# hinike/cairo

Measured on AMD Instinct MI355X. Metric: encoded Mpixels/s (p-frame, q=16) at 1/2/4/8 MI355X; bit-exact vs ref, higher is better.
Workload: dtype int16

## Files before the change

### cairo_amd/__init__.py

```python
from __future__ import annotations

import ctypes
import os
from dataclasses import dataclass

import numpy as np

_HERE = os.path.dirname(os.path.abspath(__file__))
LIB_PATH = os.path.join(_HERE, "_lib", "libcairo_amd.so")

BLOCK_DESC = np.dtype(
    [
        ("block_type", "<u4"),
        ("prediction_target", "u1"),
        ("pad", "u1"),
        ("motion_x", "<i2"),
        ("motion_y", "<i2"),
        ("sp_pred", "u1"),
        ("sp_amount", "u1"),
        ("sp_index", "u1"),
        ("q_index", "u1"),
        ("variance", "<i2"),
    ]
)
# ... 373 lines not shown
    def __del__(self):
        try:
            self.close()
        except Exception:
            pass

    @property
    def stages(self) -> int:
        return int(self.L.cairo_ctx_stages(self.h))

    def submit(self, rgb, index: int, inter: bool, quality: int, on_device: bool = False,
               fmt: int = FMT_RGB24, pitch: int = 0, src_size=None, crop=None) -> int:
        t = ctypes.c_int()
        if src_size is not None or crop is not None:
            if src_size is None:
                raise ValueError("crop needs src_size")
            s = _source(src_size, crop)
            ptr = _scaled_source_ptr(rgb, on_device, fmt, src_size, pitch)
            _ck(self.L.cairo_ctx_submit_scaled(self.h, ptr, fmt, pitch, ctypes.byref(s), index, int(inter), quality,
                                               ctypes.byref(t)), "cairo_ctx_submit_scaled")
            return t.value
        ptr = rgb if on_device else _host_frame_fmt(rgb, fmt, self.width, self.height, pitch)
        if fmt == FMT_RGB24 and not pitch:
            _ck(
                self.L.cairo_ctx_submit(self.h, ptr, int(on_device), index, int(inter), quality, ctypes.byref(t)),
                "cairo_ctx_submit",
            )
        else:
            _ck(self.L.cairo_ctx_submit_fmt(self.h, ptr, int(on_device), fmt, pitch, index, int(inter), quality,
                                            ctypes.byref(t)), "cairo_ctx_submit_fmt")
        if not on_device:
            self._keep[t.value] = rgb
        return t.value

    def wait(self, ticket: int, copy: bool = True) -> FrameOutputs:
        r = _FrameResult()
        st = self.L.cairo_ctx_wait(self.h, ticket, ctypes.byref(r))
        if st != EVX_SUCCESS:
            raise CairoError("cairo_ctx_wait", st, self.timeout_info() if st == EVX_ERROR_HARDWAREFAIL else None)
        self._keep.pop(ticket, None)
        return self._outputs(r, copy)

    ACCT_FIELDS = ("coder_tasks", "coder_total", "coder_group_wait", "coder_window", "coder_search", "coder_inter",
                   "coder_dequeue", "coder_mbs", "helper_tasks", "helper_total", "helper_wait", "helper_deblock",
                   "helper_search", "helper_catchup", "helper_dequeue", "helper_chunks",
                   "win_bytes", "win_spec_unused_bytes", "zero_mv_bytes", "gran_poll_bytes", "rec_poll_bytes",
                   "win_stages", "searched_tasks", "inter_tasks", "coder_xform", "coder_publish", "coder_drain",
                   "coder_vm0", "coder_records", "coder_prebarrier", "coder_store_tail",
                   "search_eval", "search_barrier", "search_select", "subpel_eval", "subpel_barrier",
                   "subpel_select", "db_inputs", "db_filter", "db_write",
                   "search_passes", "search_mbs_2pass", "search_mbs_3pass", "search_mbs_4pass",
                   "coder_xform_copy", "coder_copy_mbs", "coder_xform_coded", "coder_coded_mbs",
                   "helper_carry", "carry_bytes",
                   "coder_prologue_fresh", "coder_prologue_records", "helper_group_start")

    def read_acct(self, reset: bool = False) -> dict:
        w = np.zeros(len(self.ACCT_FIELDS), np.uint64)
        _ck(self.L.cairo_ctx_read_acct(self.h, _ptr(w), len(w), int(reset)), "cairo_ctx_read_acct")
        return {k: int(w[i]) for i, k in enumerate(self.ACCT_FIELDS)}

    def timeout_info(self) -> dict | None:
        w = np.zeros(16, np.int32)
        _ck(self.L.cairo_ctx_timeout_info(self.h, _ptr(w), 16), "cairo_ctx_timeout_info")
        if not w[0]:
            return None
        d = {k: int(w[i]) for i, k in enumerate(TIMEOUT_FIELDS)}
        d["kind"] = WAIT_KINDS.get(d["kind"], str(d["kind"]))
        d["seen"] = (d.pop("seen_hi") & 0xFFFFFFFF) << 32 | (d.pop("seen_lo") & 0xFFFFFFFF)
        return d

    def _outputs(self, r, copy: bool) -> FrameOutputs:
        ny, nc = r.wa * r.ha, (r.wa // 2) * (r.ha // 2)
        mbs = r.wmb * r.hmb
        has_coef = bool(r.coef_y)
        feed = _view(r.feed, np.uint32, (r.feed_bits + 31) // 32) if r.feed_status == FEED_VALID else None
        out = FrameOutputs(
            _view(r.block_table, BLOCK_DESC, mbs),
            _view(r.coef_y, np.int16, ny).reshape(r.ha, r.wa) if has_coef else None,
            _view(r.coef_u, np.int16, nc).reshape(r.ha // 2, r.wa // 2) if has_coef else None,
            _view(r.coef_v, np.int16, nc).reshape(r.ha // 2, r.wa // 2) if has_coef else None,
            feed, int(r.feed_bits), int(r.feed_status),
        )
        if copy:
            cp = lambda a: None if a is None else a.copy()
            out = FrameOutputs(cp(out.table), cp(out.coef_y), cp(out.coef_u), cp(out.coef_v), cp(out.feed),
                               out.feed_bits, out.feed_status)
        return out

    def set_outputs(self, outputs: int) -> None:
        _ck(self.L.cairo_ctx_set_outputs(self.h, outputs), "cairo_ctx_set_outputs")

    def fetch_coef(self, ticket: int):
        r = _FrameResult()
        _ck(self.L.cairo_ctx_fetch_coef(self.h, ticket, ctypes.byref(r)), "cairo_ctx_fetch_coef")
        ny, nc = self.wa * self.ha, (self.wa // 2) * (self.ha // 2)
        return (_view(r.coef_y, np.int16, ny).reshape(self.ha, self.wa).copy(),
                _view(r.coef_u, np.int16, nc).reshape(self.ha // 2, self.wa // 2).copy(),
                _view(r.coef_v, np.int16, nc).reshape(self.ha // 2, self.wa // 2).copy())

    def set_metrics(self, sse: bool = True, ssim: bool = True, keep_recon: bool = False, flags: int | None = None) -> None:
        if flags is None:
            flags = (METRIC_SSE if sse else 0) | (METRIC_SSIM if ssim else 0) | (KEEP_RECON if keep_recon else 0)
        _ck(self.L.cairo_ctx_set_metrics(self.h, flags), "cairo_ctx_set_metrics")

    def frame_metrics(self, ticket: int) -> dict:
        m = _FrameMetrics()
        _ck(self.L.cairo_ctx_frame_metrics(self.h, ticket, ctypes.byref(m)), "cairo_ctx_frame_metrics")
# ... 531 lines not shown
```

### cairo_amd/csrc/kernels.h

```cpp
#pragma once

#include <hip/hip_runtime.h>
#include <stddef.h>
#include <stdint.h>

#include "evx_defs.h"

namespace cairo {

struct PlaneSet {
  int16_t* y;
  int16_t* u;
  int16_t* v;
};

__host__ __device__ inline PlaneSet ring_slot(int16_t* base, size_t slot_elems, int wa, int ha,
                                              int k) {
  PlaneSet p;
  p.y = base + (size_t)k * slot_elems;
  p.u = p.y + (size_t)wa * ha;
  p.v = p.u + (size_t)(wa / 2) * (ha / 2);
  return p;
}

// ... 3 lines not shown
__host__ __device__ inline uint32_t pack_inter_desc(const BlockDesc& d) {
  return (d.block_type & 7u) | ((uint32_t)(d.prediction_target & 3) << 3) | ((uint32_t)(d.sp_pred & 1) << 5) |
         ((uint32_t)(d.sp_amount & 1) << 6) | ((uint32_t)(d.sp_index & 15) << 7) |
         (((uint32_t)d.motion_x & 0x7Fu) << 11) | (((uint32_t)d.motion_y & 0x7Fu) << 18);
}
__host__ __device__ inline BlockDesc unpack_inter_desc(uint32_t w) {
  BlockDesc d;
  d.block_type = w & 7u;
  d.prediction_target = (uint8_t)((w >> 3) & 3);
  d.pad = 0;
  d.sp_pred = (uint8_t)((w >> 5) & 1);
  d.sp_amount = (uint8_t)((w >> 6) & 1);
  d.sp_index = (uint8_t)((w >> 7) & 15);
  d.motion_x = (int16_t)((int32_t)(w << 14) >> 25);
  d.motion_y = (int16_t)((int32_t)(w << 7) >> 25);
  d.q_index = 0;
  d.variance = 0;
  return d;
}

constexpr int kStampPhases = 12;
constexpr int kDbStamps = 256;
constexpr int kIStamps = 12;
__host__ __device__ inline size_t stamp_frame_words(int wmb, int hmb) {
  return (size_t)wmb * hmb * kStampPhases + (size_t)hmb * kDbStamps;
}

struct TimeoutInfo {
  static constexpr int kKind = 0;
  static constexpr int kEpoch = 1;
  static constexpr int kIndex = 2;
  static constexpr int kRow = 3;
  static constexpr int kMember = 4;
  static constexpr int kNeed = 5;
  static constexpr int kOn = 6;
  static constexpr int kSeenLo = 7;
  static constexpr int kSeenHi = 8;
  static constexpr int kClaim = 9;
  static constexpr int kWords = 16;
};
enum TimeoutKind : int32_t {
  kWaitRecords = 1,
  kWaitGranule = 2,
  kWaitPrevProgress = 3,
  kWaitRowAbove = 4,
  kWaitBatch = 5,
  kWaitInjected = 6,
  kWaitHostMark = 9,
};

#ifndef CAIRO_ACCT
#define CAIRO_ACCT 0
#endif
constexpr int kAcctShards = 64, kAcctWords = 53;
struct Acct {
  static constexpr int kCoderTasks = 0, kCoderTotal = 1, kCoderGroupWait = 2, kCoderWindow = 3, kCoderSearch = 4,
                       kCoderInter = 5, kCoderDequeue = 6, kCoderMBs = 7;
  static constexpr int kHelperTasks = 8, kHelperTotal = 9, kHelperWait = 10, kHelperDeblock = 11, kHelperSearch = 12,
                       kHelperCatchup = 13, kHelperDequeue = 14, kHelperChunks = 15;
  static constexpr int kWinBytes = 16, kWinSpecUnused = 17, kZeroMvBytes = 18, kGranPollBytes = 19,
                       kRecPollBytes = 20, kWinStages = 21, kSearchedTasks = 22, kInterTasks = 23;
  static constexpr int kCoderXform = 24, kCoderPublish = 25, kCoderDrain = 26;
  static constexpr int kCoderVm0 = 27, kCoderRecords = 28, kCoderPreBarrier = 29;
  static constexpr int kCoderStoreTail = 30;
  static constexpr int kSrchEval = 31, kSrchBarrier = 32, kSrchSelect = 33, kSubEval = 34, kSubBarrier = 35,
                       kSubSelect = 36;
  static constexpr int kDbInputs = 37, kDbFilter = 38, kDbWrite = 39;
  static constexpr int kSrchPasses = 40, kSrchPasses2 = 41, kSrchPasses3 = 42, kSrchPasses4 = 43;
  static constexpr int kCoderXformCopy = 44, kCoderCopyMBs = 45, kCoderXformCoded = 46, kCoderCodedMBs = 47;
  static constexpr int kHelperCarry = 48, kCarryBytes = 49;
  static constexpr int kCoderProFresh = 50, kCoderProRecords = 51, kHelperGroupStart = 52;
};

#ifndef CAIRO_MAX_BATCH
#define CAIRO_MAX_BATCH 48
#endif
constexpr int kMaxBatch = CAIRO_MAX_BATCH;
constexpr int kMaxGroup = 16;
constexpr int kMaxPush = kMaxRing;

struct FrameDesc {
  const uint8_t* rgb;
  const uint8_t* host_rgb;
  int index;
  int inter;
  int quality;
  uint32_t epoch;
  int slot;
  int decode;
  PlaneSet recon[kMaxRing];
  PlaneSet stale;
  PlaneSet coef;
  PlaneSet push[kMaxPush];
  int npush;
  PlaneSet coef_prev;
  uint64_t* progress;
  const uint64_t* prev_progress;
  const uint64_t* prev2_progress;
  int sys;
  int member;
  const BlockDesc* host_table;
  const int16_t* host_coef;
};

struct alignas(64) FrameArgs {
  int wa, ha;
  int wmb, hmb;
  uint32_t epoch;
  int nrec;
  BlockDesc* inter_desc;
  PlaneSet in;
  uint64_t* granules;
  PlaneSet stale;
  int ring;
  int pad1;
  int32_t* inter_done;
  int ng;
  int sys;
  int nref;
  int inter;
  uint64_t* acct;
  PlaneSet recon[kMaxRing];
  BlockDesc* table;
  int quality;
// ... 140 lines not shown
```

### cairo_amd/csrc/kernels.hip

```cpp
#include "kernels.h"

namespace cairo {

typedef const __attribute__((address_space(4))) FrameArgs FA;
#define RECON_AT(a, k)                                                                   \
  ((k) == 1 ? planes((a).recon[1]) : (k) == 2 ? planes((a).recon[2]) : (k) == 3 ? planes((a).recon[3]) \
                                                                              : planes((a).recon[0]))
__host__ __device__ inline PlaneSet planes(const __attribute__((address_space(4))) PlaneSet& p) {
  PlaneSet r;
  r.y = p.y;
  r.u = p.u;
  r.v = p.v;
  return r;
}


__constant__ int16_t kLut8[64] = {
    128, 128,  128,  128,  128,  128,  128,  128,
    126, 106,  71,   25,   -25,  -71,  -106, -126,
    118, 49,   -49,  -118, -118, -49,  49,   118,
    106, -25,  -126, -71,  71,   126,  25,   -106,
    91,  -91,  -91,  91,   91,   -91,  -91,  91,
    71,  -126, 25,   106,  -106, -25,  126,  -71,
    49,  -118, 118,  -49,  -49,  118,  -118, 49,
// ... 43 lines not shown
  }
  __syncthreads();
}


__device__ __forceinline__ int wave_sum(int v) {
  v += __builtin_amdgcn_mov_dpp(v, 0x128, 0xF, 0xF, false);
  v += __builtin_amdgcn_mov_dpp(v, 0x124, 0xF, 0xF, false);
  v += __builtin_amdgcn_mov_dpp(v, 0x122, 0xF, 0xF, false);
  v += __builtin_amdgcn_mov_dpp(v, 0x121, 0xF, 0xF, false);
  return __builtin_amdgcn_readlane(v, 0) + __builtin_amdgcn_readlane(v, 16) +
         __builtin_amdgcn_readlane(v, 32) + __builtin_amdgcn_readlane(v, 48);
}
__device__ __forceinline__ int wave_max(int v) {
  v = max(v, __builtin_amdgcn_mov_dpp(v, 0x128, 0xF, 0xF, false));
  v = max(v, __builtin_amdgcn_mov_dpp(v, 0x124, 0xF, 0xF, false));
  v = max(v, __builtin_amdgcn_mov_dpp(v, 0x122, 0xF, 0xF, false));
  v = max(v, __builtin_amdgcn_mov_dpp(v, 0x121, 0xF, 0xF, false));
  return max(max(__builtin_amdgcn_readlane(v, 0), __builtin_amdgcn_readlane(v, 16)),
             max(__builtin_amdgcn_readlane(v, 32), __builtin_amdgcn_readlane(v, 48)));
}

__device__ __forceinline__ int lane_id() { return threadIdx.x & 63; }

__device__ __forceinline__ void trace(int32_t* t, int k, int v) {
  if (t && threadIdx.x == 0)
    __hip_atomic_store(&t[blockIdx.x * 4 + k], v, __ATOMIC_RELAXED, __HIP_MEMORY_SCOPE_SYSTEM);
}

__device__ __forceinline__ int16_t* pick(const PlaneSet& p, int pl) {
  int16_t* const y = p.y;
  int16_t* const u = p.u;
  int16_t* const v = p.v;
  return pl == 0 ? y : (pl == 1 ? u : v);
}

__device__ __forceinline__ int fresh(int v) {
  asm volatile("" : "+v"(v));
  return v;
}

__device__ __forceinline__ int uni(int v) { return __builtin_amdgcn_readfirstlane(v); }

__device__ __forceinline__ void stamp(uint64_t* stamps, int mb, int k) {
  if (stamps && threadIdx.x == 0) stamps[(size_t)mb * kStampPhases + k] = __builtin_amdgcn_s_memrealtime();
}
__device__ __forceinline__ void stamp(FA& a, int mb, int k) { stamp(a.stamps, mb, k); }

__device__ __forceinline__ uint64_t acct_now() { return CAIRO_ACCT ? __builtin_amdgcn_s_memrealtime() : 0; }
__device__ __forceinline__ void acct_add(uint64_t* acct, int k, uint64_t v) {
  if (CAIRO_ACCT && acct && threadIdx.x == 0)
    __hip_atomic_fetch_add(&acct[(blockIdx.x & (kAcctShards - 1)) * kAcctWords + k], v, __ATOMIC_RELAXED,
                           __HIP_MEMORY_SCOPE_AGENT);
}

#ifndef CAIRO_ASM_MARKS
#define CAIRO_ASM_MARKS 0
#endif
#if CAIRO_ASM_MARKS
#define ASM_MARK(s) asm volatile("; cairo-mark " s)
#else
#define ASM_MARK(s) ((void)0)
#endif

__device__ __forceinline__ uint64_t tagged(uint32_t epoch, int cols) {
  return ((uint64_t)epoch << 32) | (uint32_t)cols;
}
__device__ __forceinline__ uint64_t progress_at(const uint64_t* p) {
  return __hip_atomic_load(p, __ATOMIC_RELAXED, __HIP_MEMORY_SCOPE_AGENT);
}
__device__ __forceinline__ uint64_t progress_peer(bool sys, const uint64_t* p) {
  return sys ? __hip_atomic_load(p, __ATOMIC_RELAXED, __HIP_MEMORY_SCOPE_SYSTEM)
             : __hip_atomic_load(p, __ATOMIC_RELAXED, __HIP_MEMORY_SCOPE_AGENT);
}
__device__ __forceinline__ void acquire_fence(bool sys) {
  if (sys)
    __builtin_amdgcn_fence(__ATOMIC_ACQUIRE, "");
  else
    __builtin_amdgcn_fence(__ATOMIC_ACQUIRE, "agent");
}

constexpr int kWaitSleep = 2, kGranSleep = 1;

__device__ __attribute__((noinline)) void report_timeout(int32_t* err, int32_t* sticky, int kind, uint32_t epoch,
                                                         int index, int row, int member, int need, int on,
                                                         uint64_t seen) {
  __hip_atomic_store(err, 1, __ATOMIC_RELAXED, __HIP_MEMORY_SCOPE_AGENT);
  int32_t none = 0;
  if (!__hip_atomic_compare_exchange_strong(sticky + TimeoutInfo::kClaim, &none, 1, __ATOMIC_RELAXED,
                                            __ATOMIC_RELAXED, __HIP_MEMORY_SCOPE_AGENT))
    return;
  const int32_t w[8] = {(int32_t)epoch, index, row, member, need, on, (int32_t)(uint32_t)seen, (int32_t)(seen >> 32)};
  for (int k = 0; k < 8; k++) __hip_atomic_store(sticky + 1 + k, w[k], __ATOMIC_RELAXED, __HIP_MEMORY_SCOPE_AGENT);
  __hip_atomic_store(sticky + TimeoutInfo::kKind, kind, __ATOMIC_RELEASE, __HIP_MEMORY_SCOPE_SYSTEM);
}
__device__ __forceinline__ void report_timeout(FA& a, int kind, int row, int need, int on, uint64_t seen) {
  report_timeout(a.err, a.sticky, kind, a.epoch, a.index, row, a.member, need, on, seen);
}

__device__ __forceinline__ void wait_records(FA& a, int row, int group) {
  int32_t* word = &a.inter_done[row * a.ng + group];
  int v = __hip_atomic_load(word, __ATOMIC_RELAXED, __HIP_MEMORY_SCOPE_AGENT);
  if (v >= a.nref) return;
  uint64_t t0 = __builtin_amdgcn_s_memrealtime();
  while ((v = __hip_atomic_load(word, __ATOMIC_RELAXED, __HIP_MEMORY_SCOPE_AGENT)) < a.nref) {
    if (__hip_atomic_load(a.err, __ATOMIC_RELAXED, __HIP_MEMORY_SCOPE_AGENT)) return;
// ... 517 lines not shown
        row0_min(live && sad < kSadGate ? (((uint32_t)sad << 5) | (uint32_t)(c + 1)) : 0xFFFFFFFFu);
    if (k < ((uint32_t)min(s.sad, 1 << 26) << 5)) w = (int)(k & 31) - 1;
  }
  if (w >= 0) {
    const int n = w >> 1, k9 = n < 4 ? n : n + 1;
    s.sp_en = 1;
    s.sp_amt = w & 1;
    s.sp_idx = frac_index(k9 % 3 - 1, k9 / 3 - 1);
    s.sad = __builtin_amdgcn_readlane(sad, w);
    s.mad = __builtin_amdgcn_readlane(mad, w);
  }
}

__device__ __forceinline__ bool in_frame(int x, int y, int wa, int ha) {
  return x >= 0 && x <= wa - kMB && y >= 0 && y <= ha - kMB;
}

__device__ __forceinline__ BlockDesc make_desc(const Sel& s, int px, int py, int thr, bool intra,
                                               int target) {
  BlockDesc d;
  uint32_t t = intra ? kIntra : 0u;
  if (s.bx != px || s.by != py || s.sp_en) t |= kMotion;
  if (s.mad < thr) t |= kCopy;
  d.block_type = t;
  d.prediction_target = (uint8_t)target;
  d.pad = 0;
  d.motion_x = (int16_t)(s.bx - px);
  d.motion_y = (int16_t)(s.by - py);
  d.sp_pred = (uint8_t)s.sp_en;
  d.sp_amount = (uint8_t)s.sp_amt;
  d.sp_index = (uint8_t)s.sp_idx;
  d.q_index = 0;
  d.variance = 0;
  return d;
}


constexpr int kLvl1Rows = 77, kLvl1Cols = 112;

__device__ __forceinline__ int wg_broadcast(volatile int* slot, int v) {
  if (threadIdx.x == 0) *slot = v;
  __syncthreads();
  const int r = *slot;
  __syncthreads();
  return r;
}

struct DbLds;
struct DbState;
__device__ __forceinline__ bool deblock_chunk_ready(FA& a, int r, const DbState& st);
__device__ __forceinline__ void deblock_chunk(FA& a, int r, DbLds& D, DbState& st, bool known_ready = false);
__device__ __forceinline__ bool deblock_pending(FA& a, const DbState& st);

template <bool kDeblock = true>
__device__ __forceinline__ void helper_wait(FA& a, int back, int r, int rr, int need, DbLds& D, DbState& st,
                                            int* flag) {
  volatile int* vflag = flag;
  const uint64_t* pp = back == 1 ? a.prev_progress : a.prev2_progress;
  uint64_t t0 = 0;
  const uint64_t ta = acct_now();
  uint64_t tdb = 0;
  for (;;) {
    int d = 0;
    if (threadIdx.x == 0) {
      const uint64_t pv = pp ? progress_peer(a.sys, pp + rr) : ~0ull;
      const bool dbr = kDeblock && deblock_pending(a, st) && deblock_chunk_ready(a, r, st);
      if (a.inject && r == min(1, a.hmb - 1)) {
        report_timeout(a, kWaitInjected, r, need, rr | (back << 16), pv);
        d = 1;
      } else if (pv >= tagged(a.epoch - back, need)) {
        d = 1;
      } else if (dbr) {
        d = 2;
      } else {
        const uint64_t now = __builtin_amdgcn_s_memrealtime();
        if (!t0) t0 = now;
        __builtin_amdgcn_s_sleep(1);
        if (__hip_atomic_load(a.err, __ATOMIC_RELAXED, __HIP_MEMORY_SCOPE_AGENT)) {
          d = 1;
        } else if (now - t0 > 200000000ull) {
          report_timeout(a, kWaitPrevProgress, r, need, rr | (back << 16), pv);
          d = 1;
        }
      }
    }
    d = wg_broadcast(vflag, d);
    if (d == 1) break;
    if (kDeblock && d == 2) {
      const uint64_t tb = acct_now();
      deblock_chunk(a, r, D, st, true);
      tdb += acct_now() - tb;
    }
  }
  if (threadIdx.x == 0) {
    acquire_fence(a.sys);
    asm volatile("s_waitcnt vmcnt(0)" ::: "memory");
  }
  __syncthreads();
  acct_add(a.acct, Acct::kHelperWait, acct_now() - ta - tdb);
}

struct InterLds {
  Window win;
  int need[4];
  int full;
  int lvl2[6][4];
  alignas(16) int16_t src[4][384];
  int zsad[kMaxRing][4], zmad[kMaxRing][4];
};

__device__ __forceinline__ void group_source(FA& a, int r, int g, InterLds& L) {
  const int wave = threadIdx.x >> 6, lane = threadIdx.x & 63, x = 4 * g + wave;
  if (x >= a.wmb || lane >= 48) return;
  const PlaneSet in = planes(a.in);
  const int px = x * kMB, py = r * kMB;
  const int16_t* gsrc;
  if (lane < 32) {
    gsrc = in.y + (size_t)(py + (lane >> 1)) * a.wa + px + 8 * (lane & 1);
  } else {
    const int k = lane - 32;
    gsrc = pick(in, 1 + (k >> 3)) + (size_t)((py >> 1) + (k & 7)) * (a.wa >> 1) + (px >> 1);
  }
  *(uint4*)&L.src[wave][8 * lane] = *(const uint4*)gsrc;
}

__device__ __forceinline__ void src_dma(const PlaneSet& in, int wa, int x, int r, int16_t* dst) {
  const int lane = threadIdx.x;
  if (lane >= 48) return;
  const int px = x * kMB, py = r * kMB;
  const int16_t* gsrc = lane < 32 ? in.y + (size_t)(py + (lane >> 1)) * wa + px + 8 * (lane & 1)
                                  : pick(in, 1 + ((lane - 32) >> 3)) +
                                        (size_t)((py >> 1) + (lane & 7)) * (wa >> 1) + (px >> 1);
  __builtin_amdgcn_global_load_lds((const void*)gsrc, (lds_void*)dst, 16, 0, 0);
}
__device__ __forceinline__ void src_dma(FA& a, int x, int r, int16_t* dst) { src_dma(planes(a.in), a.wa, x, r, dst); }

__device__ __forceinline__ Px6 src_px_lds(const InterLds& L, int wave) {
  const int l = threadIdx.x & 63;
  const int16_t* m = L.src[wave];
  Px6 p;
  const int16_t* y = &m[(l >> 2) * 16 + (l & 3) * 4];
  p.y0 = y[0], p.y1 = y[1], p.y2 = y[2], p.y3 = y[3];
  p.u = m[256 + (l >> 3) * 8 + (l & 7)];
  p.v = m[320 + (l >> 3) * 8 + (l & 7)];
  return p;
}
__device__ __forceinline__ SrcRow src_rows_lds(const InterLds& L, int wave, int i) {
  const uint32_t* m = (const uint32_t*)L.src[wave];
  SrcRow s;
#pragma unroll
  for (int k = 0; k < 8; k++) s.y[k] = m[i * 8 + k] ^ 0x80008000u;
  const int co = (i >> 1) * 4 + (i & 1) * 2;
  s.u[0] = m[128 + co] ^ 0x80008000u, s.u[1] = m[128 + co + 1] ^ 0x80008000u;
  s.v[0] = m[160 + co] ^ 0x80008000u, s.v[1] = m[160 + co + 1] ^ 0x80008000u;
  return s;
}

__device__ __forceinline__ void zero_mv_older(FA& a, int r, int g, InterLds& L) {
  const int wave = threadIdx.x >> 6, x = 4 * g + wave;
  acct_add(a.acct, Acct::kZeroMvBytes, 768ull * (a.nref - 1) * (uint64_t)min(4, a.wmb - 4 * g));
  if (x >= a.wmb) return;
  const int px = x * kMB, py = r * kMB;
  const Px6 src = src_px_lds(L, wave);
  Px6 ref[kMaxRing - 1];
#pragma unroll
  for (int off = 2; off < kMaxRing; off++)
    if (off <= a.nref) ref[off - 1] = px_from_planes(RECON_AT(a, off), a.wa, px, py);
#pragma unroll
  for (int off = 2; off < kMaxRing; off++) {
    if (off > a.nref) break;
    int sad, mad;
    sad_mad(src, ref[off - 1], sad, mad);
    if ((threadIdx.x & 63) == 0) L.zsad[off][wave] = sad, L.zmad[off][wave] = mad;
  }
}

__device__ __forceinline__ int inter_need_cols(FA& a, int g, int level) {
  return min(64 * g + (level == 1 ? 80 : 96), a.wa);
}

#ifndef CAIRO_CODER_CARRY
#define CAIRO_CODER_CARRY 0
#endif

typedef uint32_t u32x4 __attribute__((ext_vector_type(4)));
typedef __attribute__((address_space(1))) u32x4 gbl_u32x4;
__device__ __forceinline__ void store16_through(bool sys, int16_t* p, u32x4 v) {
  if (sys)
    asm volatile("global_store_dwordx4 %0, %1, off sc0 sc1" ::"v"(p), "v"(v) : "memory");
  else
    asm volatile("global_store_dwordx4 %0, %1, off sc1" ::"v"(p), "v"(v) : "memory");
}

__device__ __forceinline__ bool carry_group(FA& a, int r, int g) {
  if (CAIRO_CODER_CARRY) return false;
  const PlaneSet dst = planes(a.coef), src = planes(a.coef_prev);
  if (dst.y == src.y) return false;
  const uint64_t t0 = acct_now();
  const int t = threadIdx.x;
  int pl, row, x, col;
  if (t < 128) {
    pl = 0, row = r * kMB + (t >> 3), x = 4 * g + ((t & 7) >> 1), col = 4 * g * kMB + 8 * (t & 7);
  } else {
    const int k = t - 128;
    pl = 1 + (k >> 5), row = r * (kMB / 2) + ((k & 31) >> 2), x = 4 * g + (k & 3), col = x * (kMB / 2);
  }
  if (t < 192 && x < a.wmb) {
    const size_t off = (size_t)row * (pl ? a.wa >> 1 : a.wa) + col;
    const u32x4 v = *(const gbl_u32x4*)(pick(src, pl) + off);
    store16_through(a.sys, pick(dst, pl) + off, v);
  }
  acct_add(a.acct, Acct::kHelperCarry, acct_now() - t0);
  acct_add(a.acct, Acct::kCarryBytes, 768ull * (uint64_t)min(4, a.wmb - 4 * g));
  return true;
}

__device__ __forceinline__ void inter_task(FA& a0, int r, int g, int off, InterLds& L, DbLds& D, DbState& st,
                                           int* flag, uint64_t* is, bool carried = false) {
  FA& a = *opaque_view(&a0);
  ASM_MARK("group_start begin");
  const uint64_t tg0 = acct_now();
  const int wave = uni(threadIdx.x >> 6);
  const int x = 4 * g + wave;
  const bool valid = x < a.wmb;
  const int px = x * kMB, py = r * kMB, mb = r * a.wmb + x;
  const int mbs = a.wmb * a.hmb;
  const int thr = (a.quality >> 2) + 1;
  const PlaneSet ref = RECON_AT(a, off);
  Sel s;
  Px6 src;
  s.bx = px;
  s.by = py;
  s.ssd = INT32_MAX;
  s.sp_idx = s.sp_amt = s.sp_en = 0;
  s.sad = s.mad = 0;
  SrcRow srow;
  const int ox = 4 * g * kMB - 32, oy = py - 32;
  if (valid) {
    src = src_px_lds(L, wave);
    srow = src_rows_lds(L, wave, threadIdx.x & 15);
    if (off >= 2) {
      s.sad = L.zsad[off][wave], s.mad = L.zmad[off][wave];
    } else {
      sad_mad(src, px_from_planes(ref, a.wa, px, py), s.sad, s.mad);
    }
  }
  const bool need = valid && s.mad >= thr && !(CAIRO_ATTR_SKIP & 8);
  if ((threadIdx.x & 63) == 0) L.need[wave] = need;
  if (threadIdx.x == 0) {
    const int back = off == 1 ? 1 : 2;
    const uint64_t* pp = back == 1 ? a.prev_progress : a.prev2_progress;
    const uint64_t want = tagged(a.epoch - back, inter_need_cols(a, g, 2));
    const uint64_t w3 = pp ? progress_peer(a.sys, pp + min(r + 3, a.hmb - 1)) : 0;
    const uint64_t w2 = pp ? progress_peer(a.sys, pp + min(r + 2, a.hmb - 1)) : 0;
    const int full = !pp || ((w3 >= want) & (w2 >= want));
    if (full && pp) {
      acquire_fence(a.sys);
      asm volatile("s_waitcnt vmcnt(0)" ::: "memory");
    }
    L.full = full;
  }
  __syncthreads();
  if (is && off == 1) is[3] = __builtin_amdgcn_s_memrealtime();
  acct_add(a.acct, Acct::kInterTasks, 1);
  acct_add(a.acct, Acct::kZeroMvBytes, (off == 1 ? 768ull : 0ull) * (uint64_t)min(4, a.wmb - 4 * g));
  if (L.need[0] | L.need[1] | L.need[2] | L.need[3]) {
    const bool full = L.full != 0;
    acct_add(a.acct, Acct::kSearchedTasks, 1);
    acct_window(a.acct, 0, full ? kWinL : kLvl1Rows, 0, full ? kWinLW : kLvl1Cols);
    acct_add(a.acct, Acct::kHelperGroupStart, acct_now() - tg0);
    ASM_MARK("group_start end");
    stage_window(L.win, ref, a.wa, a.ha, ox, oy, 0, full ? kWinL : kLvl1Rows, 0, full ? kWinLW : kLvl1Cols);
    __syncthreads();
    if (is && off == 1) is[4] = __builtin_amdgcn_s_memrealtime();
    bool lvl2c = full, lvl2r = full;
    bool lvl2_open = true;
    for (int si = 0; si < 6; si++) {
      const int step = si < 5 ? kRadius >> si : 1;
      if (!lvl2r && lvl2_open) {
        const int rem = si < 5 ? 2 * step : 1;
        const int want = need ? (s.by + step - oy > kLvl1Rows - kMB) * 2 + (!lvl2c && s.bx + step - ox > kLvl1Cols - kMB)
                              : 0;
        const int may = need && (s.by + rem - oy > kLvl1Rows - kMB || (!lvl2c && s.bx + rem - ox > kLvl1Cols - kMB));
        if ((threadIdx.x & 63) == 0) L.lvl2[si][wave] = want | (may << 2);
        __syncthreads();
        const int m4 = L.lvl2[si][0] | L.lvl2[si][1] | L.lvl2[si][2] | L.lvl2[si][3];
        const int m = m4 & 3;
        lvl2_open = (m4 >> 2) != 0;
        if (m) {
          if (is) is[5] = __builtin_amdgcn_s_memrealtime();
          helper_wait<false>(a, off == 1 ? 1 : 2, r, min(r + ((m & 2) ? 3 : 2), a.hmb - 1), inter_need_cols(a, g, 2),
                             D, st, flag);
          if (m & 2) stage_window(L.win, ref, a.wa, a.ha, ox, oy, kLvl1Rows, kWinL, 0, kWinLW);
          if (!lvl2c) stage_window(L.win, ref, a.wa, a.ha, ox, oy, 0, kLvl1Rows, kLvl1Cols, kWinLW);
          if (m & 2) acct_window(a.acct, kLvl1Rows, kWinL, 0, kWinLW);
          if (!lvl2c) acct_window(a.acct, 0, kLvl1Rows, kLvl1Cols, kWinLW);
          __syncthreads();
          if (is) is[6] = __builtin_amdgcn_s_memrealtime(), is[7] += (m & 2) ? 0x10000 : 1;
          lvl2c = true;
          lvl2r = (m & 2) != 0;
        }
      }
      if (is && off == 1 && (si == 1 || si == 5)) is[si == 1 ? 8 : 9] = __builtin_amdgcn_s_memrealtime();
      if (!need) continue;
      if (si < 5) {
        const int bx = s.bx, by = s.by;
        const int lane = threadIdx.x & 63, gi = lane & 15, grp = lane >> 4;
        const int my_pass = gi < 4 ? 0 : 1, my_grp = gi < 4 ? gi : gi - 5;
        int sadv = s.sad, madv = s.mad;
#pragma unroll
        for (int pass = 0; pass < 2; pass++) {
          const int c = 4 * pass + grp + (pass > 0);
          const int cx = bx + (c % 3 - 1) * step, cy = by + (c / 3 - 1) * step;
          const bool ok = in_frame(cx, cy, a.wa, a.ha);
          int sad, mad;
          inter_cand_row(L.win, (ok ? cx : bx) - ox, (ok ? cy : by) - oy, gi, srow, thr, sad, mad);
          const int from = (16 * (my_grp & 3)) << 2;
          const int vs = __builtin_amdgcn_ds_bpermute(from, sad), vm = __builtin_amdgcn_ds_bpermute(from, mad);
          if (my_pass == pass && gi != 4) sadv = vs, madv = vm;
        }
        {
          const int cx = bx + (gi % 3 - 1) * step, cy = by + (gi / 3 - 1) * step;
          select_int(s, gi < 9 && in_frame(cx, cy, a.wa, a.ha), cx, cy, sadv, madv, px, py, thr, lane);
        }
      } else {
        const Px6 best = px_from_window_b(L.win, s.bx - ox, s.by - oy);
        s.sp_idx = s.sp_amt = s.sp_en = 0;
        const int bx = s.bx, by = s.by;
        const uint32_t sb0 = src.y0 + 0x8000, sb1 = src.y1 + 0x8000, sb2 = src.y2 + 0x8000, sb3 = src.y3 + 0x8000,
                       sbu = src.u + 0x8000, sbv = src.v + 0x8000;
        const uint32_t b30 = 3 * best.y0, b31 = 3 * best.y1, b32 = 3 * best.y2, b33 = 3 * best.y3, b3u = 3 * best.u,
                       b3v = 3 * best.v;
#pragma unroll
        for (int n = 0; n < 8; n++) {
          const int k9 = n < 4 ? n : n + 1, i = k9 % 3 - 1, j = k9 / 3 - 1, tx = bx + i, ty = by + j;
          const bool ok = in_frame(tx, ty, a.wa, a.ha);
          if (!ok) continue;
          const Px6 nb = px_from_window_b(L.win, tx - ox, ty - oy);
          const int idx = frac_index(i, j);
#pragma unroll
          for (int q = 0; q < 2; q++) {
            const uint32_t d0 = absdiff_b(sb0, q ? lerp_quarter_bb3(b30, nb.y0) : lerp_half_bb(best.y0, nb.y0)),
                           d1 = absdiff_b(sb1, q ? lerp_quarter_bb3(b31, nb.y1) : lerp_half_bb(best.y1, nb.y1)),
                           d2 = absdiff_b(sb2, q ? lerp_quarter_bb3(b32, nb.y2) : lerp_half_bb(best.y2, nb.y2)),
                           d3 = absdiff_b(sb3, q ? lerp_quarter_bb3(b33, nb.y3) : lerp_half_bb(best.y3, nb.y3)),
                           du = absdiff_b(sbu, q ? lerp_quarter_bb3(b3u, nb.u) : lerp_half_bb(best.u, nb.u)),
                           dv = absdiff_b(sbv, q ? lerp_quarter_bb3(b3v, nb.v) : lerp_half_bb(best.v, nb.v));
            const int lsum = (int)(d0 + d1 + d2 + d3);
            const int lmax = (int)max(max(max(d0, d1), d2), max(max(d3, du), dv));
            const bool copy = s.mad < thr;
            const bool mad_lt = __ballot(lmax >= (copy ? s.mad : thr)) == 0;
            int sad = 0;
            bool acc;
            if (copy) {
              acc = mad_lt;
            } else {
              sad = wave_sum(lsum);
              acc = (sad < s.sad && sad < kSadGate) || mad_lt;
            }
            if (acc) {
              s.sp_en = 1;
              s.sp_amt = q;
              s.sp_idx = idx;
              s.sad = copy ? wave_sum(lsum) : sad;
              s.mad = wave_max(lmax);
            }
          }
        }
      }
    }
  } else if (carried) {
    asm volatile("s_waitcnt vmcnt(0)" ::: "memory");
    __syncthreads();
  }
  if (is && off == 1) is[10] = __builtin_amdgcn_s_memrealtime();
  if (valid && (threadIdx.x & 63) == 0) {
    const BlockDesc d = make_desc(s, px, py, thr, false, off);
    uint64_t* rec = (uint64_t*)&a.inter_desc[(off - 1) * mbs + mb];
    const uint64_t tag = (uint64_t)a.epoch << 32;
    gran_st(rec, tag | pack_inter_desc(d));
    gran_st(rec + 1, tag | (uint32_t)s.sad);
  }
  asm volatile("s_waitcnt lgkmcnt(0)\n\ts_barrier" ::: "memory");
}


constexpr int kMBElems = 384;
typedef short int8v __attribute__((ext_vector_type(8)));

__device__ __forceinline__ void elem_coords(int e, int x, int y, int& plane, int& ex, int& ey) {
  int b = e >> 6, r = (e >> 3) & 7, c = e & 7;
  if (b < 4) {
    plane = 0;
    ex = x + (b & 1) * 8 + c;
    ey = y + (b >> 1) * 8 + r;
  } else {
    plane = b - 3;
    ex = (x >> 1) + c;
    ey = (y >> 1) + r;
  }
}


__device__ __forceinline__ int8v load_row8(const int16_t* p) {
  return *(const int8v*)p;
}

__device__ __forceinline__ int fdct_lane(int16_t* sa, int16_t* sb, int lane, int16_t x) {
  const int r8 = lane >> 3, c8 = lane & 7;
  sa[lane] = x;
  __builtin_amdgcn_wave_barrier();
  {
    const int8v row = load_row8(&sa[r8 * 8]), lut = load_row8(&sLut8[c8 * 8]);
    int t = 0;
#pragma unroll
    for (int k = 0; k < 8; k++) t += row[k] * lut[k];
    t = c8 == 0 ? (t * 45) / 128 : t / 2;
    sb[c8 * 8 + r8] = (int16_t)rdiv(t, 128);
  }
  __builtin_amdgcn_wave_barrier();
  const int8v col = load_row8(&sb[c8 * 8]), lut = load_row8(&sLut8[r8 * 8]);
  int t = 0;
#pragma unroll
  for (int k = 0; k < 8; k++) t += col[k] * lut[k];
  t = r8 == 0 ? (t * 45) / 128 : t / 2;
  return (int16_t)rdiv(t, 128);
}

__device__ __forceinline__ int idct_lane(int16_t* sa, int16_t* sb, int lane, int16_t d) {
  const int r8 = lane >> 3, c8 = lane & 7;
  sa[c8 * 8 + r8] = d;
  __builtin_amdgcn_wave_barrier();
  {
    const int8v col = load_row8(&sa[c8 * 8]), lut = load_row8(&sLut8T[r8 * 8]);
    int t = ((col[0] * lut[0]) * 45) / 128;
#pragma unroll
// ... 1007 lines not shown
        else wait_vmcnt<kStoresAfterCoef[3]>();
      } else {
        asm volatile("s_waitcnt vmcnt(0)" ::: "memory");
      }
      __syncthreads();
      if (tid == 0)
        gran_st(gran_at(ps.granules, ps.wmb, bx, by, kGranulesPerMB),
                ((uint64_t)tag << 32) | ((d.block_type & kCopy) ? 0x100u : 0u) | d.q_index);
      stamp(*ap, mb, 9);
      if (CAIRO_ACCT) {
        const uint64_t tx9 = acct_now();
        acct_add(ap->acct, Acct::kCoderXform, tx7 - tx5);
        const bool cpy = (type & kCopy) != 0;
        acct_add(ap->acct, cpy ? Acct::kCoderXformCopy : Acct::kCoderXformCoded, tx7 - tx5);
        acct_add(ap->acct, cpy ? Acct::kCoderCopyMBs : Acct::kCoderCodedMBs, 1);
        acct_add(ap->acct, Acct::kCoderPublish, tx8 - tx7);
        acct_add(ap->acct, Acct::kCoderDrain, tx9 - tx8);
      }
      if (ap->stamps && tid == 0) ap->stamps[(size_t)mb * kStampPhases + 11] = __builtin_amdgcn_s_memtime();
      more = bx + 1 < ps.wmb;
      ASM_MARK("mb_publish end");
    }
  }
}



struct HelperLds {
  InterLds inter;
  DbLds db;
};

struct EngineLds {
  union {
    RowLds row;
    HelperLds helper;
  } u;
  int slot;
  int flag;
};

__device__ __forceinline__ void row_helper(FA& a0, int r, HelperLds& L, int* flag, int32_t* tr) {
  FA& a = a0;
  const int tid = threadIdx.x;
  const int nch = db_chunks(a);
  volatile int* vflag = flag;
  DbState st{0, 0, 0, 8};
  for (int g = 0; g < a0.ng; g++) {
    FA& a = *opaque_view(&a0);
    trace(tr, 1, g);
    trace(tr, 2, (int)a.epoch * 1000 + r);
    uint64_t* is = a.istamps && tid == 0 ? a.istamps + (size_t)(r * a.ng + g) * kIStamps : nullptr;
    if (is) is[0] = __builtin_amdgcn_s_memrealtime(), is[3] = is[4] = is[5] = is[6] = is[7] = is[8] = is[9] = is[10] = 0;
    if (a.inter) group_source(a, r, g, L.inter);
    if (a.inter && a.nref >= 2) {
      helper_wait(a, 2, r, min(r + 2, a.hmb - 1), inter_need_cols(a, g, 1), L.db, st, flag);
      const uint64_t ts = acct_now();
      zero_mv_older(a, r, g, L.inter);
      for (int off = 2; off <= a.nref; off++) inter_task(a, r, g, off, L.inter, L.db, st, flag, is);
      acct_add(a.acct, Acct::kHelperSearch, acct_now() - ts);
    }
    helper_wait(a, 1, r, min(r + 2, a.hmb - 1), inter_need_cols(a, g, 1), L.db, st, flag);
    if (is) is[1] = __builtin_amdgcn_s_memrealtime();
    trace(tr, 3, 50);
    if (a.inter) {
      const bool carried = carry_group(a, r, g);
      const uint64_t ts = acct_now();
      inter_task(a, r, g, 1, L.inter, L.db, st, flag, is, carried);
      acct_add(a.acct, Acct::kHelperSearch, acct_now() - ts);
    } else if (tid == 0) {
      __builtin_amdgcn_fence(__ATOMIC_RELEASE, "agent");
      asm volatile("s_waitcnt vmcnt(0)" ::: "memory");
      __hip_atomic_fetch_add(&a.inter_done[r * a.ng + g], 1, __ATOMIC_RELAXED, __HIP_MEMORY_SCOPE_AGENT);
    }
    if (is) is[2] = __builtin_amdgcn_s_memrealtime();
    int caught = 0;
    const uint64_t tc = acct_now();
    uint64_t tcdb = 0;
    for (;;) {
      int d = 0;
      if (tid == 0) d = st.k < nch && deblock_chunk_ready(a, r, st);
      if (!wg_broadcast(vflag, d)) break;
      const uint64_t tb = acct_now();
      deblock_chunk(a, r, L.db, st, true);
      tcdb += acct_now() - tb;
      caught++;
    }
    acct_add(a.acct, Acct::kHelperCatchup, acct_now() - tc - tcdb);
    if (is) is[11] = ((uint64_t)caught << 32) | (uint32_t)(__builtin_amdgcn_s_memrealtime() - is[2]);
  }
  trace(tr, 1, 1000);
  while (st.k < nch) {
    trace(tr, 3, 60000 + st.k);
    int d = 0;
    if (tid == 0) {
      const uint64_t t0 = __builtin_amdgcn_s_memrealtime();
      while (!(d = deblock_chunk_ready(a, r, st))) {
        if (__hip_atomic_load(a.err, __ATOMIC_RELAXED, __HIP_MEMORY_SCOPE_AGENT) ||
            __builtin_amdgcn_s_memrealtime() - t0 > 100000000ull)
          break;
        __builtin_amdgcn_s_sleep(kWaitSleep);
      }
    }
    deblock_chunk(a, r, L.db, st, wg_broadcast(vflag, d) != 0);
  }
  trace(tr, 3, 100000);
  if (a.stamps && tid == 0) {
    uint64_t* ds = a.stamps + (size_t)a.wmb * a.hmb * kStampPhases + (size_t)r * kDbStamps;
    ds[kDbStamps - 1] = st.busy;
  }
}


constexpr int kPrioLevel = 2;

__device__ __forceinline__ bool is_helper(int b, int nh, int n) {
  return ((b + 1) * nh) / n > (b * nh) / n;
}

constexpr int kSteal = 2;
__device__ __forceinline__ int next_task(const EngineArgs& e, int pool, int lab, EngineLds& L, bool& prev) {
  const int ptotal = e.ptotal;
// ... 311 lines not shown
```

Before: 7346.

## Fold full-window progress check into helper wait and trim idle inter-task barriers

The helper wait now also samples progress rows r+2/r+3 when it succeeds, recording whether the full search window is ready so inter tasks can skip their own polling. The zero-motion need flags for older refs are computed in zero_mv_older, which lets those tasks skip polling and the trailing barrier when nothing needs searching. For ref1, the coefficient carry load/store and the zero-MV reference loads are issued together to overlap their latency. New accounting counters are added as well, compiled out by default. The aim is fewer serialized progress polls and workgroup barriers per group, at the cost of more complex control flow and an extra barrier in zero_mv_older.

```diff
diff --git a/cairo_amd/__init__.py b/cairo_amd/__init__.py
--- a/cairo_amd/__init__.py
+++ b/cairo_amd/__init__.py
@@ -449,7 +449,10 @@
                    "search_passes", "search_mbs_2pass", "search_mbs_3pass", "search_mbs_4pass",
                    "coder_xform_copy", "coder_copy_mbs", "coder_xform_coded", "coder_coded_mbs",
                    "helper_carry", "carry_bytes",
-                   "coder_prologue_fresh", "coder_prologue_records", "helper_group_start")
+                   "coder_prologue_fresh", "coder_prologue_records", "helper_group_start",
+                   "start_older_searched", "start_ref1_searched", "start_older_idle", "start_ref1_idle",
+                   "older_searched", "older_idle", "ref1_idle",
+                   "flag_set", "fallback_polls", "fallback_full", "lvl2_runs", "idle_groups", "idle_group_time")
 
     def read_acct(self, reset: bool = False) -> dict:
         w = np.zeros(len(self.ACCT_FIELDS), np.uint64)
diff --git a/cairo_amd/csrc/kernels.h b/cairo_amd/csrc/kernels.h
--- a/cairo_amd/csrc/kernels.h
+++ b/cairo_amd/csrc/kernels.h
@@ -79,7 +79,7 @@
 #ifndef CAIRO_ACCT
 #define CAIRO_ACCT 0
 #endif
-constexpr int kAcctShards = 64, kAcctWords = 53;
+constexpr int kAcctShards = 64, kAcctWords = 66;
 struct Acct {
   static constexpr int kCoderTasks = 0, kCoderTotal = 1, kCoderGroupWait = 2, kCoderWindow = 3, kCoderSearch = 4,
                        kCoderInter = 5, kCoderDequeue = 6, kCoderMBs = 7;
@@ -97,6 +97,10 @@
   static constexpr int kCoderXformCopy = 44, kCoderCopyMBs = 45, kCoderXformCoded = 46, kCoderCodedMBs = 47;
   static constexpr int kHelperCarry = 48, kCarryBytes = 49;
   static constexpr int kCoderProFresh = 50, kCoderProRecords = 51, kHelperGroupStart = 52;
+  static constexpr int kStartOlderSearched = 53, kStartRef1Searched = 54, kStartOlderIdle = 55, kStartRef1Idle = 56,
+                       kOlderSearched = 57, kOlderIdle = 58, kRef1Idle = 59;
+  static constexpr int kFlagSet = 60, kFallbackPolls = 61, kFallbackFull = 62, kLvl2Runs = 63;
+  static constexpr int kIdleGroups = 64, kIdleGroupTime = 65;
 };
 
 #ifndef CAIRO_MAX_BATCH
diff --git a/cairo_amd/csrc/kernels.hip b/cairo_amd/csrc/kernels.hip
--- a/cairo_amd/csrc/kernels.hip
+++ b/cairo_amd/csrc/kernels.hip
@@ -119,6 +119,13 @@
   if (CAIRO_ACCT && acct && threadIdx.x == 0)
     __hip_atomic_fetch_add(&acct[(blockIdx.x & (kAcctShards - 1)) * kAcctWords + k], v, __ATOMIC_RELAXED,
                            __HIP_MEMORY_SCOPE_AGENT);
+}
+
+#ifndef CAIRO_ACCT_START
+#define CAIRO_ACCT_START CAIRO_ACCT
+#endif
+__device__ __forceinline__ void acct_start(uint64_t* acct, int k, uint64_t v) {
+  if (CAIRO_ACCT_START) acct_add(acct, k, v);
 }
 
 #ifndef CAIRO_ASM_MARKS
@@ -742,9 +749,14 @@
 __device__ __forceinline__ void deblock_chunk(FA& a, int r, DbLds& D, DbState& st, bool known_ready = false);
 __device__ __forceinline__ bool deblock_pending(FA& a, const DbState& st);
 
+__device__ __forceinline__ int inter_need_cols(FA& a, int g, int level) {
+  return min(64 * g + (level == 1 ? 80 : 96), a.wa);
+}
+
 template <bool kDeblock = true>
 __device__ __forceinline__ void helper_wait(FA& a, int back, int r, int rr, int need, DbLds& D, DbState& st,
-                                            int* flag) {
+                                            int* flag, int* full2 = nullptr, bool want_full = false,
+                                            int g = 0) {
   volatile int* vflag = flag;
   const uint64_t* pp = back == 1 ? a.prev_progress : a.prev2_progress;
   uint64_t t0 = 0;
@@ -754,12 +766,22 @@
     int d = 0;
     if (threadIdx.x == 0) {
       const uint64_t pv = pp ? progress_peer(a.sys, pp + rr) : ~0ull;
+      uint64_t w3 = ~0ull, w2 = ~0ull;
+      if (want_full && pp) {
+        w3 = progress_peer(a.sys, pp + min(r + 3, a.hmb - 1));
+        w2 = progress_peer(a.sys, pp + min(r + 2, a.hmb - 1));
+      }
       const bool dbr = kDeblock && deblock_pending(a, st) && deblock_chunk_ready(a, r, st);
       if (a.inject && r == min(1, a.hmb - 1)) {
         report_timeout(a, kWaitInjected, r, need, rr | (back << 16), pv);
         d = 1;
+        if (want_full) *full2 = 0;
       } else if (pv >= tagged(a.epoch - back, need)) {
         d = 1;
+        if (want_full) {
+          const uint64_t want = tagged(a.epoch - back, inter_need_cols(a, g, 2));
+          *full2 = (w3 >= want) & (w2 >= want);
+        }
       } else if (dbr) {
         d = 2;
       } else {
@@ -772,6 +794,7 @@
           report_timeout(a, kWaitPrevProgress, r, need, rr | (back << 16), pv);
           d = 1;
         }
+        if (d && want_full) *full2 = 0;
       }
     }
     d = wg_broadcast(vflag, d);
@@ -797,6 +820,8 @@
   int lvl2[6][4];
   alignas(16) int16_t src[4][384];
   int zsad[kMaxRing][4], zmad[kMaxRing][4];
+  int zneed[kMaxRing][4];
+  int wfull[2];
 };
 
 __device__ __forceinline__ void group_source(FA& a, int r, int g, InterLds& L) {
@@ -849,24 +874,29 @@
 __device__ __forceinline__ void zero_mv_older(FA& a, int r, int g, InterLds& L) {
   const int wave = threadIdx.x >> 6, x = 4 * g + wave;
   acct_add(a.acct, Acct::kZeroMvBytes, 768ull * (a.nref - 1) * (uint64_t)min(4, a.wmb - 4 * g));
-  if (x >= a.wmb) return;
-  const int px = x * kMB, py = r * kMB;
-  const Px6 src = src_px_lds(L, wave);
-  Px6 ref[kMaxRing - 1];
-#pragma unroll
-  for (int off = 2; off < kMaxRing; off++)
-    if (off <= a.nref) ref[off - 1] = px_from_planes(RECON_AT(a, off), a.wa, px, py);
-#pragma unroll
-  for (int off = 2; off < kMaxRing; off++) {
-    if (off > a.nref) break;
-    int sad, mad;
-    sad_mad(src, ref[off - 1], sad, mad);
-    if ((threadIdx.x & 63) == 0) L.zsad[off][wave] = sad, L.zmad[off][wave] = mad;
-  }
-}
-
-__device__ __forceinline__ int inter_need_cols(FA& a, int g, int level) {
-  return min(64 * g + (level == 1 ? 80 : 96), a.wa);
+  if (x < a.wmb) {
+    const int px = x * kMB, py = r * kMB;
+    const int thr = (a.quality >> 2) + 1;
+    const Px6 src = src_px_lds(L, wave);
+    Px6 ref[kMaxRing - 1];
+#pragma unroll
+    for (int off = 2; off < kMaxRing; off++)
+      if (off <= a.nref) ref[off - 1] = px_from_planes(RECON_AT(a, off), a.wa, px, py);
+#pragma unroll
+    for (int off = 2; off < kMaxRing; off++) {
+      if (off > a.nref) break;
+      int sad, mad;
+      sad_mad(src, ref[off - 1], sad, mad);
+      if ((threadIdx.x & 63) == 0) {
+        L.zsad[off][wave] = sad, L.zmad[off][wave] = mad;
+        L.zneed[off][wave] = mad >= thr && !(CAIRO_ATTR_SKIP & 8);
+      }
+    }
+  } else if ((threadIdx.x & 63) == 0) {
+#pragma unroll
+    for (int off = 2; off < kMaxRing; off++) L.zneed[off][wave] = 0;
+  }
+  __syncthreads();
 }
 
 #ifndef CAIRO_CODER_CARRY
@@ -875,6 +905,8 @@
 
 typedef uint32_t u32x4 __attribute__((ext_vector_type(4)));
 typedef __attribute__((address_space(1))) u32x4 gbl_u32x4;
+typedef uint32_t u32x2 __attribute__((ext_vector_type(2)));
+typedef u32x2 u32x2_u __attribute__((aligned(2)));
 __device__ __forceinline__ void store16_through(bool sys, int16_t* p, u32x4 v) {
   if (sys)
     asm volatile("global_store_dwordx4 %0, %1, off sc0 sc1" ::"v"(p), "v"(v) : "memory");
@@ -882,30 +914,30 @@
     asm volatile("global_store_dwordx4 %0, %1, off sc1" ::"v"(p), "v"(v) : "memory");
 }
 
-__device__ __forceinline__ bool carry_group(FA& a, int r, int g) {
-  if (CAIRO_CODER_CARRY) return false;
-  const PlaneSet dst = planes(a.coef), src = planes(a.coef_prev);
-  if (dst.y == src.y) return false;
-  const uint64_t t0 = acct_now();
+__device__ __forceinline__ bool carry_wanted(FA& a) {
+  return !CAIRO_CODER_CARRY && planes(a.coef).y != planes(a.coef_prev).y;
+}
+__device__ __forceinline__ ptrdiff_t carry_chunk(FA& a, int r, int g, int& pl) {
   const int t = threadIdx.x;
-  int pl, row, x, col;
+  int row, x, col;
   if (t < 128) {
     pl = 0, row = r * kMB + (t >> 3), x = 4 * g + ((t & 7) >> 1), col = 4 * g * kMB + 8 * (t & 7);
   } else {
     const int k = t - 128;
     pl = 1 + (k >> 5), row = r * (kMB / 2) + ((k & 31) >> 2), x = 4 * g + (k & 3), col = x * (kMB / 2);
   }
-  if (t < 192 && x < a.wmb) {
-    const size_t off = (size_t)row * (pl ? a.wa >> 1 : a.wa) + col;
-    const u32x4 v = *(const gbl_u32x4*)(pick(src, pl) + off);
-    store16_through(a.sys, pick(dst, pl) + off, v);
-  }
-  acct_add(a.acct, Acct::kHelperCarry, acct_now() - t0);
-  acct_add(a.acct, Acct::kCarryBytes, 768ull * (uint64_t)min(4, a.wmb - 4 * g));
-  return true;
-}
-
-__device__ __forceinline__ void inter_task(FA& a0, int r, int g, int off, InterLds& L, DbLds& D, DbState& st,
+  if (t >= 192 || x >= a.wmb) return -1;
+  return (ptrdiff_t)((size_t)row * (pl ? a.wa >> 1 : a.wa) + col);
+}
+__device__ __forceinline__ u32x4 carry_load(FA& a, int pl, ptrdiff_t off) {
+  return *(const gbl_u32x4*)(pick(planes(a.coef_prev), pl) + off);
+}
+__device__ __forceinline__ void carry_store(FA& a, int pl, ptrdiff_t off, u32x4 v) {
+  store16_through(a.sys, pick(planes(a.coef), pl) + off, v);
+}
+
+template <bool kRef1>
+__device__ __forceinline__ bool inter_task(FA& a0, int r, int g, int off, InterLds& L, DbLds& D, DbState& st,
                                            int* flag, uint64_t* is, bool carried = false) {
   FA& a = *opaque_view(&a0);
   ASM_MARK("group_start begin");
@@ -926,39 +958,99 @@
   s.sad = s.mad = 0;
   SrcRow srow;
   const int ox = 4 * g * kMB - 32, oy = py - 32;
-  if (valid) {
-    src = src_px_lds(L, wave);
-    srow = src_rows_lds(L, wave, threadIdx.x & 15);
-    if (off >= 2) {
+  const uint64_t* pp = kRef1 ? a.prev_progress : a.prev2_progress;
+  const uint64_t want = tagged(a.epoch - (kRef1 ? 1 : 2), inter_need_cols(a, g, 2));
+  const bool wf = uni(L.wfull[kRef1 ? 0 : 1]) != 0 || !pp;
+  bool need = false;
+  bool any, full = wf;
+  if (kRef1) {
+    int cpl = 0;
+    const ptrdiff_t coff = carried ? carry_chunk(a, r, g, cpl) : -1;
+    const uint64_t tc0 = acct_now();
+    u32x4 cv = {0, 0, 0, 0};
+    if (coff >= 0) cv = carry_load(a, cpl, coff);
+    u32x2 zy = {0, 0};
+    int zu = 0, zv = 0;
+    if (valid) {
+      const int l = lane_id();
+      const size_t co = (size_t)((py >> 1) + (l >> 3)) * (a.wa >> 1) + (px >> 1) + (l & 7);
+      zy = *(const u32x2_u*)&ref.y[(size_t)(py + (l >> 2)) * a.wa + px + (l & 3) * 4];
+      zu = ref.u[co], zv = ref.v[co];
+    }
+    const bool poll = threadIdx.x == 0 && !wf;
+    uint64_t w3 = 0, w2 = 0;
+    if (poll) {
+      w3 = progress_peer(a.sys, pp + min(r + 3, a.hmb - 1));
+      w2 = progress_peer(a.sys, pp + min(r + 2, a.hmb - 1));
+    }
+    asm volatile("" : "+v"(cv), "+v"(zy), "+v"(zu), "+v"(zv), "+v"(w3), "+v"(w2));
+    if (coff >= 0) carry_store(a, cpl, coff, cv);
+    Px6 zref;
+    zref.y0 = (int16_t)zy.x, zref.y1 = (int16_t)(zy.x >> 16), zref.y2 = (int16_t)zy.y, zref.y3 = (int16_t)(zy.y >> 16);
+    zref.u = zu, zref.v = zv;
+    if (carried) {
+      acct_add(a.acct, Acct::kHelperCarry, acct_now() - tc0);
+      acct_add(a.acct, Acct::kCarryBytes, 768ull * (uint64_t)min(4, a.wmb - 4 * g));
+    }
+    if (valid) {
+      src = src_px_lds(L, wave);
+      srow = src_rows_lds(L, wave, threadIdx.x & 15);
+      sad_mad(src, zref, s.sad, s.mad);
+    }
+    need = valid && s.mad >= thr && !(CAIRO_ATTR_SKIP & 8);
+    if ((threadIdx.x & 63) == 0) L.need[wave] = need;
+    if (threadIdx.x == 0) {
+      int f = wf;
+      if (poll) {
+        f = (w3 >= want) & (w2 >= want);
+        if (f) {
+          acquire_fence(a.sys);
+          asm volatile("s_waitcnt vmcnt(0)" ::: "memory");
+        }
+        acct_start(a.acct, Acct::kFallbackFull, f);
+      }
+      L.full = f;
+    }
+    __syncthreads();
+    any = uni(L.need[0] | L.need[1] | L.need[2] | L.need[3]) != 0;
+    full = uni(L.full) != 0;
+    if (is) is[3] = __builtin_amdgcn_s_memrealtime();
+  } else {
+    any = uni(L.zneed[off][0] | L.zneed[off][1] | L.zneed[off][2] | L.zneed[off][3]) != 0;
+    if (valid) {
+      src = src_px_lds(L, wave);
+      srow = src_rows_lds(L, wave, threadIdx.x & 15);
       s.sad = L.zsad[off][wave], s.mad = L.zmad[off][wave];
-    } else {
-      sad_mad(src, px_from_planes(ref, a.wa, px, py), s.sad, s.mad);
-    }
-  }
-  const bool need = valid && s.mad >= thr && !(CAIRO_ATTR_SKIP & 8);
-  if ((threadIdx.x & 63) == 0) L.need[wave] = need;
-  if (threadIdx.x == 0) {
-    const int back = off == 1 ? 1 : 2;
-    const uint64_t* pp = back == 1 ? a.prev_progress : a.prev2_progress;
-    const uint64_t want = tagged(a.epoch - back, inter_need_cols(a, g, 2));
-    const uint64_t w3 = pp ? progress_peer(a.sys, pp + min(r + 3, a.hmb - 1)) : 0;
-    const uint64_t w2 = pp ? progress_peer(a.sys, pp + min(r + 2, a.hmb - 1)) : 0;
-    const int full = !pp || ((w3 >= want) & (w2 >= want));
-    if (full && pp) {
-      acquire_fence(a.sys);
-      asm volatile("s_waitcnt vmcnt(0)" ::: "memory");
-    }
-    L.full = full;
-  }
-  __syncthreads();
-  if (is && off == 1) is[3] = __builtin_amdgcn_s_memrealtime();
+      need = L.zneed[off][wave] != 0;
+    }
+    if (any && !wf) {
+      if (threadIdx.x == 0) {
+        const uint64_t w3 = progress_peer(a.sys, pp + min(r + 3, a.hmb - 1));
+        const uint64_t w2 = progress_peer(a.sys, pp + min(r + 2, a.hmb - 1));
+        const int f = (w3 >= want) & (w2 >= want);
+        if (f) {
+          acquire_fence(a.sys);
+          asm volatile("s_waitcnt vmcnt(0)" ::: "memory");
+        }
+        acct_start(a.acct, Acct::kFallbackFull, f);
+        L.full = f;
+      }
+      __syncthreads();
+      full = uni(L.full) != 0;
+    }
+  }
   acct_add(a.acct, Acct::kInterTasks, 1);
-  acct_add(a.acct, Acct::kZeroMvBytes, (off == 1 ? 768ull : 0ull) * (uint64_t)min(4, a.wmb - 4 * g));
-  if (L.need[0] | L.need[1] | L.need[2] | L.need[3]) {
-    const bool full = L.full != 0;
+  acct_add(a.acct, Acct::kZeroMvBytes, (kRef1 ? 768ull : 0ull) * (uint64_t)min(4, a.wmb - 4 * g));
+  if (kRef1 || any) {
+    acct_start(a.acct, Acct::kFlagSet, wf);
+    acct_start(a.acct, Acct::kFallbackPolls, !wf);
+  }
+  if (any) {
     acct_add(a.acct, Acct::kSearchedTasks, 1);
     acct_window(a.acct, 0, full ? kWinL : kLvl1Rows, 0, full ? kWinLW : kLvl1Cols);
     acct_add(a.acct, Acct::kHelperGroupStart, acct_now() - tg0);
+    acct_start(a.acct, kRef1 ? Acct::kStartRef1Searched : Acct::kStartOlderSearched, acct_now() - tg0);
+    acct_start(a.acct, Acct::kOlderSearched, kRef1 ? 0 : 1);
     ASM_MARK("group_start end");
     stage_window(L.win, ref, a.wa, a.ha, ox, oy, 0, full ? kWinL : kLvl1Rows, 0, full ? kWinLW : kLvl1Cols);
     __syncthreads();
@@ -979,6 +1071,7 @@
         lvl2_open = (m4 >> 2) != 0;
         if (m) {
           if (is) is[5] = __builtin_amdgcn_s_memrealtime();
+          acct_start(a.acct, Acct::kLvl2Runs, 1);
           helper_wait<false>(a, off == 1 ? 1 : 2, r, min(r + ((m & 2) ? 3 : 2), a.hmb - 1), inter_need_cols(a, g, 2),
                              D, st, flag);
           if (m & 2) stage_window(L.win, ref, a.wa, a.ha, ox, oy, kLvl1Rows, kWinL, 0, kWinLW);
@@ -1063,6 +1156,10 @@
     asm volatile("s_waitcnt vmcnt(0)" ::: "memory");
     __syncthreads();
   }
+  if (!any) {
+    acct_start(a.acct, kRef1 ? Acct::kStartRef1Idle : Acct::kStartOlderIdle, acct_now() - tg0);
+    acct_start(a.acct, kRef1 ? Acct::kRef1Idle : Acct::kOlderIdle, 1);
+  }
   if (is && off == 1) is[10] = __builtin_amdgcn_s_memrealtime();
   if (valid && (threadIdx.x & 63) == 0) {
     const BlockDesc d = make_desc(s, px, py, thr, false, off);
@@ -1071,7 +1168,8 @@
     gran_st(rec, tag | pack_inter_desc(d));
     gran_st(rec + 1, tag | (uint32_t)s.sad);
   }
-  asm volatile("s_waitcnt lgkmcnt(0)\n\ts_barrier" ::: "memory");
+  if (kRef1 || any) asm volatile("s_waitcnt lgkmcnt(0)\n\ts_barrier" ::: "memory");
+  return any;
 }
 
 
@@ -2185,22 +2283,30 @@
     trace(tr, 2, (int)a.epoch * 1000 + r);
     uint64_t* is = a.istamps && tid == 0 ? a.istamps + (size_t)(r * a.ng + g) * kIStamps : nullptr;
     if (is) is[0] = __builtin_amdgcn_s_memrealtime(), is[3] = is[4] = is[5] = is[6] = is[7] = is[8] = is[9] = is[10] = 0;
+    const uint64_t tgrp = acct_now();
+    bool searched = false;
     if (a.inter) group_source(a, r, g, L.inter);
     if (a.inter && a.nref >= 2) {
-      helper_wait(a, 2, r, min(r + 2, a.hmb - 1), inter_need_cols(a, g, 1), L.db, st, flag);
+      helper_wait(a, 2, r, min(r + 2, a.hmb - 1), inter_need_cols(a, g, 1), L.db, st, flag, &L.inter.wfull[1], true,
+                  g);
       const uint64_t ts = acct_now();
       zero_mv_older(a, r, g, L.inter);
-      for (int off = 2; off <= a.nref; off++) inter_task(a, r, g, off, L.inter, L.db, st, flag, is);
+      for (int off = 2; off <= a.nref; off++)
+        searched |= inter_task<false>(a, r, g, off, L.inter, L.db, st, flag, is);
       acct_add(a.acct, Acct::kHelperSearch, acct_now() - ts);
     }
-    helper_wait(a, 1, r, min(r + 2, a.hmb - 1), inter_need_cols(a, g, 1), L.db, st, flag);
+    helper_wait(a, 1, r, min(r + 2, a.hmb - 1), inter_need_cols(a, g, 1), L.db, st, flag,
+                &L.inter.wfull[0], a.inter != 0, g);
     if (is) is[1] = __builtin_amdgcn_s_memrealtime();
     trace(tr, 3, 50);
     if (a.inter) {
-      const bool carried = carry_group(a, r, g);
       const uint64_t ts = acct_now();
-      inter_task(a, r, g, 1, L.inter, L.db, st, flag, is, carried);
+      searched |= inter_task<true>(a, r, g, 1, L.inter, L.db, st, flag, is, carry_wanted(a));
       acct_add(a.acct, Acct::kHelperSearch, acct_now() - ts);
+      if (!searched) {
+        acct_start(a.acct, Acct::kIdleGroups, 1);
+        acct_start(a.acct, Acct::kIdleGroupTime, acct_now() - tgrp);
+      }
     } else if (tid == 0) {
       __builtin_amdgcn_fence(__ATOMIC_RELEASE, "agent");
       asm volatile("s_waitcnt vmcnt(0)" ::: "memory");
```

Result: faster. 7440, median of 6 (+1.3%).
